# shenzebang/PDE-inverse-problem

Hardware: AMD Instinct MI355X
Metric: particle-steps/sec + achieved HBM GB/s; recovered-drift L2 error (higher is better)
Workload: dtype f32; 1 GPU; C2 kinetic OU d=4: EM simulate (traj+tau+last, fused moments) + KFP residual value_and_grad; dim=4, n_steps=100, particles_per_gpu=2097152, particles_total=2097152, parallelism=dp1

## Files before the change

include/pdeinv.h:

```cpp
#ifndef PDEINV_H
#define PDEINV_H

#include <stddef.h>
#include <stdint.h>

#ifdef __cplusplus
extern "C" {
#endif

#define PDEINV_ABI_VERSION 10
#define PDEINV_MAX_DIM 16
#define PDEINV_MAX_PARAMS 256

typedef enum {
  PDEINV_OK = 0,
  PDEINV_ERR_INVALID = -1,
  PDEINV_ERR_UNSUPPORTED = -2,
  PDEINV_ERR_HIP = -3
} pdeinv_status;

typedef enum {
  PDEINV_POT_QUADRATIC = 0,
  PDEINV_POT_GMM = 1,
  PDEINV_POT_MEANFIELD_QUADRATIC = 2,
  PDEINV_POT_NONE = 3
} pdeinv_potential_kind;

typedef struct {
  int32_t kind;
  int32_t n_centers;
  float sigma;
  int32_t has_center;
  const float* params;
} pdeinv_potential;

typedef struct {
  int64_t n_particles;
  int64_t particle_offset;
  int32_t dim;
  int32_t n_steps;
  float dt;
  float gamma;
  float noise_scale;
  int32_t random_shift;
  uint64_t seed;
  uint32_t counter_offset;
  int64_t ld_z0;
  pdeinv_potential potential;
  const float* d_noise;
  const float* d_shift_u;
  const float* d_meanfield;
} pdeinv_sde_desc;

int pdeinv_moment_len(int m);
size_t pdeinv_sde_workspace_bytes(const pdeinv_sde_desc* desc);
int pdeinv_sde_simulate(const pdeinv_sde_desc* desc, const float* d_z0, float* d_traj,
                        float* d_tau, float* d_last, void* d_workspace, double* d_moments,
                        void* stream);

size_t pdeinv_mf_workspace_bytes(const pdeinv_sde_desc* desc);
int pdeinv_mf_step(const pdeinv_sde_desc* desc, int32_t s, const float* d_z, float* d_z_out,
                   float* d_tau_row, const float* d_tau0, const double* d_xbar_sum,
                   void* d_workspace, double* d_xsum, void* stream);
int64_t pdeinv_mf_sums_len(const pdeinv_sde_desc* desc);
size_t pdeinv_mf_sums_workspace_bytes(const pdeinv_sde_desc* desc);
int pdeinv_mf_sums(const pdeinv_sde_desc* desc, const float* d_z0, void* d_workspace, double* d_sums,
                   void* stream);
int pdeinv_mf_mean_path(const pdeinv_sde_desc* desc, const double* d_sums, float* d_xbar, double* d_xsum,
                        void* stream);
size_t pdeinv_sde_simulate_mf_next_workspace_bytes(const pdeinv_sde_desc* desc);
int pdeinv_sde_simulate_mf_next(const pdeinv_sde_desc* desc, const float* d_z0, float* d_traj, float* d_tau,
                                float* d_last, const pdeinv_sde_desc* next, const float* d_z0_next,
                                void* d_workspace, double* d_sums_next, void* stream);
size_t pdeinv_sde_simulate_mf_kmv_workspace_bytes(const pdeinv_sde_desc* desc, int32_t with_next);
int pdeinv_sde_simulate_mf_kmv(const pdeinv_sde_desc* desc, const float* d_z0, float* d_traj, float* d_tau,
                               float* d_last, float gamma, const float* d_coef, double* d_mom, double* d_wstats,
                               const pdeinv_sde_desc* next, const float* d_z0_next, double* d_sums_next,
                               void* d_workspace, void* stream);
int pdeinv_sde_tau0(const pdeinv_sde_desc* desc, float* d_tau0, void* stream);

size_t pdeinv_moments_workspace_bytes(int64_t n_rows, int32_t m);
int pdeinv_moments(const float* d_z, int64_t n_rows, int32_t m, int64_t ld, void* d_workspace,
                   double* d_out, void* stream);

enum {
  PDEINV_KFP_LOSS = 0,
  PDEINV_KFP_LOSS_GT = 1,
  PDEINV_KFP_GRAD_NORM = 2,
  PDEINV_KFP_NABLA = 3,
  PDEINV_KFP_HESSIAN = 4,
  PDEINV_KFP_FRICTION = 5,
  PDEINV_KFP_NABLA_TRUE = 6,
  PDEINV_KFP_INITIAL = 7,
  PDEINV_KFP_TERMINAL = 8,
  PDEINV_KFP_NOUT = 9
};

typedef struct {
  int32_t dim;
  float gamma;
  float total_time;
  const float* tilde_F;
} pdeinv_kfp_quad_desc;

int pdeinv_residual_kfp_quadratic(const pdeinv_kfp_quad_desc* desc, const double* d_moments,
                                  const float* d_theta, float* d_out, float* d_grad,
                                  void* stream);

enum {
  PDEINV_GMM_ACC_LOSS = 0,
  PDEINV_GMM_ACC_LOSS_GT = 1,
  PDEINV_GMM_ACC_NABLA = 2,
  PDEINV_GMM_ACC_HESSIAN = 3,
  PDEINV_GMM_ACC_FRICTION = 4,
  PDEINV_GMM_ACC_NABLA_TRUE = 5,
  PDEINV_GMM_ACC_INITIAL = 6,
  PDEINV_GMM_ACC_TERMINAL = 7,
  PDEINV_GMM_NACC = 8
};

typedef struct {
  int32_t dim;
  int32_t n_centers;
  float sigma;
  int32_t n_centers_true;
  float sigma_true;
  const float* mus_true;
  float gamma;
  float c_nabla, c_hess, c_fric, c_true, c_init, c_term;
} pdeinv_kfp_gmm_desc;

size_t pdeinv_residual_kfp_gmm_workspace_bytes(const pdeinv_kfp_gmm_desc* desc, int64_t n_init,
                                               int64_t n_term, int64_t n_0T);
int pdeinv_residual_kfp_gmm(const pdeinv_kfp_gmm_desc* desc, const float* d_init,
                            int64_t n_init, int64_t ld_init, const float* d_term,
                            int64_t n_term, int64_t ld_term, const float* d_0T, int64_t n_0T,
                            int64_t ld_0T, const float* d_mus, void* d_workspace,
                            double* d_acc, void* stream);

size_t pdeinv_sde_simulate_kfp_gmm_workspace_bytes(const pdeinv_sde_desc* desc, const pdeinv_kfp_gmm_desc* res);
int pdeinv_sde_simulate_kfp_gmm(const pdeinv_sde_desc* desc, const pdeinv_kfp_gmm_desc* res, const float* d_mus,
// ... 175 lines not shown
```

pde-inverse-problem_amd/csrc/sde.hip:

```cpp
#include <math.h>
#include <stddef.h>
#include <stdlib.h>

#include <type_traits>

#include "sde_common.h"

namespace pdeinv {


template <int D>
__device__ __forceinline__ void grad_quadratic(const SdeArgs& a, const float* q, float* g) {
  if constexpr (D * D + D > 32) {
    kfloat* P = kernarg_params();
#pragma unroll
    for (int r = 0; r < D; ++r) {
      float acc = -P[D * D + r];
#pragma unroll
      for (int c = 0; c < D; ++c) acc = fmaf(P[r * D + c], q[c], acc);
      g[r] = acc;
    }
  } else {
#pragma unroll
    for (int r = 0; r < D; ++r) {
      float acc = -a.params[D * D + r];
#pragma unroll
      for (int c = 0; c < D; ++c) acc = fmaf(a.params[r * D + c], q[c], acc);
      g[r] = acc;
    }
  }
}

template <int D, int KM>
struct GmmCentres {
  GmmPairs<D, KM> g;
  __device__ __forceinline__ void load(const SdeArgs& a) {
#pragma unroll
    for (int p = 0; p < KM / 2; ++p) {
#pragma unroll
      for (int i = 0; i < D; ++i) {
        g.mu[p][i] = f32x2{2 * p < a.K ? a.params[2 * p * D + i] : 0.f, 2 * p + 1 < a.K ? a.params[(2 * p + 1) * D + i] : 0.f};
        asm volatile("" : "+v"(g.mu[p][i]));
      }
      g.c[p] = f32x2{2 * p < a.K ? a.params[kMaxGmmK * D + 2 * p] : -INFINITY,
                     2 * p + 1 < a.K ? a.params[kMaxGmmK * D + 2 * p + 1] : -INFINITY};
      asm volatile("" : "+v"(g.c[p]));
    }
  }
};




template <int D>
__device__ __forceinline__ void store_rows_staged(float* wave_dst, const float* z, float* slot,
                                                  int lane, int n_valid) {
  constexpr int M = 2 * D;
  static_assert(M % 4 == 0, "staged stores need 2d % 4 == 0");
#pragma unroll
  for (int k = 0; k < M; k += 4)
    *reinterpret_cast<f32x4*>(slot + lane * M + k) = f32x4{z[k], z[k + 1], z[k + 2], z[k + 3]};
  __builtin_amdgcn_wave_barrier();
  f32x4 v[M / 4];
#pragma unroll
  for (int k = 0; k < M / 4; ++k) v[k] = *reinterpret_cast<const f32x4*>(slot + 4 * (k * 64 + lane));
  if (n_valid == kWave) {
#pragma unroll
    for (int k = 0; k < M / 4; ++k)
      __builtin_nontemporal_store(v[k], reinterpret_cast<f32x4*>(wave_dst + 4 * (k * 64 + lane)));
  } else {
#pragma unroll
    for (int k = 0; k < M / 4; ++k) {
      const int c = k * 64 + lane;
      if (4 * c < n_valid * M) __builtin_nontemporal_store(v[k], reinterpret_cast<f32x4*>(wave_dst + 4 * c));
    }
  }
  __builtin_amdgcn_wave_barrier();
}

template <int D>
__device__ __forceinline__ void load_rows_staged(const float* wave_src, float* z, float* slot, int lane,
                                                 int n_valid) {
  constexpr int M = 2 * D;
  static_assert(M % 4 == 0, "staged loads need 2d % 4 == 0");
#pragma unroll
  for (int k = 0; k < M / 4; ++k) {
// ... 187 lines not shown
  const float sh_dt = sqrtf(a.dt) * a.ns;
  for (int s = 1; s < a.n_steps; ++s) {
    update(a.dt, sh_dt, (uint32_t)s);
    if (tr) put(tr + (int64_t)s * tr_stride);
    if (active && ta) __builtin_nontemporal_store(tau_value(tau0, s, a.dt), ta + (int64_t)s * a.N);
    if constexpr (MOM) acc.add(z);
  }

  update(h_last, sqrtf(h_last) * a.ns, (uint32_t)a.n_steps);
  if (active && last) store_row<D, kStoreNT>(last + i * M, z);
  if constexpr (NXT) {
    float* red = stage;
    const int wv = threadIdx.x >> 6;
    constexpr int NE = (128 * D + kBlock - 1) / kBlock;
    float v[NE];
#pragma unroll
    for (int t = 0; t < NE; ++t) v[t] = 0.f;
#pragma unroll
    for (int pass = 0; pass < 2; ++pass) {
      const int j0 = 2 * pass, nj = pass ? 1 : 2;
      __syncthreads();
#pragma unroll
      for (int jj = 0; jj < 2; ++jj)
        if (jj < nj) {
#pragma unroll
          for (int k = 0; k < D; ++k) red[((wv * kWave + lane) * 2 + jj) * D + k] = nacc[j0 + jj][k];
        }
      __syncthreads();
#pragma unroll
      for (int t = 0; t < NE; ++t) {
        const int e = threadIdx.x + t * kBlock;
        if (e < nx.np1 * D) {
          const int sp = e / D, k = e - sp * D;
          const int l0 = (64 * sp) / nx.np1, l1 = (64 * sp + 63) / nx.np1;
          for (int w2 = 0; w2 < kWavesPerBlock; ++w2)
            for (int l = l0; l <= l1; ++l) {
              const int jj = sp - ((l * nx.np1) >> 6) - j0;
              if (jj >= 0 && jj < nj) v[t] += red[((w2 * kWave + l) * 2 + jj) * D + k];
            }
        }
      }
    }
#pragma unroll
    for (int t = 0; t < NE; ++t) {
      const int e = threadIdx.x + t * kBlock;
      if (e < nx.np1 * D) nx.partials[(int64_t)e * nb + bid] = v[t];
    }
  }
  if constexpr (RES) {
    res_add(z, z, 2);
    constexpr int NR = PDEINV_GMM_NACC + KR * D;
    float flat[NR];
#pragma unroll
    for (int c = 0; c < PDEINV_GMM_NACC; ++c) flat[c] = racc[c];
    gmm_adjoint_flat<D, KR>(radj, lmod.mu, flat + PDEINV_GMM_NACC);
    __shared__ float rlds[kWavesPerBlock * NR];
    block_reduce_to_slab(flat, PDEINV_GMM_NACC + rf.K * D, rlds, partials, bid, nb);
  }

  if constexpr (MOM) {
    float mv[L];
    acc.finish((float)a.n_steps, w, mv);
    block_reduce_to_slab(mv, L, lds, partials + (int64_t)L * nb, bid, nb);
    MomentAcc<M> term;
    term.zero();
    term.add(z, w);
    block_reduce_to_slab(term.v, L, lds, partials + (int64_t)2 * L * nb, bid, nb);
  }
}

template <typename F>
struct first_param;
template <typename R, typename A0, typename... As>
struct first_param<R (*)(A0, As...)> {
  using type = A0;
};
static_assert(std::is_standard_layout<SdeArgs>::value, "kernarg_params(): SdeArgs must be standard-layout");
static_assert(std::is_same<first_param<decltype(&sde_simulate_kernel<4, PDEINV_POT_QUADRATIC, false, 2>)>::type,
                           SdeArgs>::value &&
                  std::is_same<first_param<decltype(&sde_simulate_kernel<8, PDEINV_POT_MEANFIELD_QUADRATIC, false, 2>)>::type,
                               SdeArgs>::value,
              "kernarg_params() reads SdeArgs::params at its kernarg offset: SdeArgs must stay the first parameter "
              "of sde_simulate_kernel");

template <int D>
__global__ __launch_bounds__(kBlock) void mf_step_kernel(SdeArgs a, int s, float tau0,
                                                         const float* __restrict__ zin,
                                                         float* __restrict__ zout,
                                                         float* __restrict__ tau_row,
                                                         const double* __restrict__ xbar_sum,
                                                         float* __restrict__ partials) {
  constexpr int M = 2 * D;
  constexpr bool kStaged = (M % 4 == 0);
  const int64_t i_raw = (int64_t)blockIdx.x * kBlock + threadIdx.x;
  const bool active = i_raw < a.N;
  const int64_t i = active ? i_raw : a.N - 1;
  const uint64_t gid = (uint64_t)(a.poff + i);
  const int lane = threadIdx.x & (kWave - 1);
  const int64_t wave_row0 = i_raw - lane;
  const int n_valid = (int)((a.N - wave_row0) < kWave ? (a.N - wave_row0) : kWave);
  __shared__ float stage[kStaged ? kBlock * M : 1];
  float* slot = stage + (threadIdx.x - lane) * M;
  float z[M] = {};
  if constexpr (kStaged) {
    if (n_valid > 0) load_rows_staged<D>(zin + wave_row0 * M, z, slot, lane, n_valid);
  } else {
#pragma unroll
    for (int k = 0; k < M; ++k) z[k] = zin[i * M + k];
  }
  const double cnt = xbar_sum[0];
  float y[D];
#pragma unroll
  for (int k = 0; k < D; ++k) y[k] = z[k] - (float)(xbar_sum[1 + k] / cnt);
  float g[D];
#pragma unroll
  for (int r = 0; r < D; ++r) {
    float acc = 0.f;
#pragma unroll
    for (int c = 0; c < D; ++c) acc = fmaf(a.params[r * D + c], y[c], acc);
    g[r] = acc;
  }
  float xi[D];
  if (a.noise) gen_normals<D, true>(a, (uint32_t)gid, (uint32_t)(gid >> 32), (uint32_t)s, i, xi);
  else gen_normals<D, false>(a, (uint32_t)gid, (uint32_t)(gid >> 32), (uint32_t)s, i, xi);
  const float h = (s == 0) ? tau0 : ((s == a.n_steps) ? a.dt - tau0 : a.dt);
  const float sh = sqrtf(h) * a.ns;
  const float gh = a.gamma * h;
#pragma unroll
  for (int k = 0; k < D; ++k) {
    const float p = z[D + k];
    const float pn = fmaf(-gh, p, fmaf(sh, xi[k], fmaf(-h, g[k], p)));
    z[D + k] = pn;
    z[k] = fmaf(h, pn, z[k]);
  }
  if constexpr (kStaged) {
    if (n_valid > 0) store_rows_staged<D>(zout + wave_row0 * M, z, slot, lane, n_valid);
  } else if (active) {
    store_row<D, kStoreNT>(zout + i * M, z);
  }
  if (active && tau_row) tau_row[i] = tau_value(tau0, s, a.dt);
  float v[1 + D];
  v[0] = active ? 1.f : 0.f;
#pragma unroll
  for (int k = 0; k < D; ++k) v[1 + k] = active ? z[k] : 0.f;
  __shared__ float lds[kWavesPerBlock * (1 + D)];
  block_reduce_to_slab(v, 1 + D, lds, partials, blockIdx.x, gridDim.x);
}

__global__ void tau0_kernel(SdeArgs a, float* __restrict__ out) {
  const int64_t i = (int64_t)blockIdx.x * kBlock + threadIdx.x;
  if (i >= a.N) return;
  const uint64_t gid = (uint64_t)(a.poff + i);
  out[i] = a.random_shift ? shift_u(a, (uint32_t)gid, (uint32_t)(gid >> 32), i) * a.dt : 0.f;
}


static int sim_grid(int64_t N) { return grid_for(N); }

}

using namespace pdeinv;

extern "C" int pdeinv_moment_len(int m) { return moment_len(m); }

extern "C" size_t pdeinv_sde_workspace_bytes(const pdeinv_sde_desc* d) {
  if (!d || d->dim < 1 || d->dim > 8 || d->n_particles <= 0) return 0;
  return (size_t)3 * moment_len(2 * d->dim) * sim_grid(d->n_particles) * sizeof(float);
}

template <int D, int POT, bool MOM, int KM = 1>
static void launch_sim(const SdeArgs& a, const float* z0, float* traj, float* tau, float* last,
                       float* ws, hipStream_t st) {
  const dim3 g(sim_grid(a.N)), b(kBlock);
  if (a.noise)
    hipLaunchKernelGGL((sde_simulate_kernel<D, POT, MOM, kStoreStaged, KM, true>), g, b, 0, st, a, z0, traj, tau,
                       last, ws);
  else
    hipLaunchKernelGGL((sde_simulate_kernel<D, POT, MOM, kStoreStaged, KM, false>), g, b, 0, st, a, z0, traj, tau,
                       last, ws);
}

template <int D> constexpr int kResMinWaves = D <= 4 ? 3 : 1;

template <int D, int KM>
static void launch_sim_res(const SdeArgs& a, const GmmResFused& rf, const float* z0, float* traj, float* tau,
                           float* last, float* ws, hipStream_t st) {
  const dim3 g(sim_grid(a.N)), b(kBlock);
  constexpr int W = kResMinWaves<D>;
  if (a.noise)
    hipLaunchKernelGGL((sde_simulate_kernel<D, PDEINV_POT_GMM, false, kStoreStaged, KM, true, W, true>), g, b, 0, st,
                       a, z0, traj, tau, last, ws, rf);
  else
    hipLaunchKernelGGL((sde_simulate_kernel<D, PDEINV_POT_GMM, false, kStoreStaged, KM, false, W, true>), g, b, 0,
                       st, a, z0, traj, tau, last, ws, rf);
}

template <int D, bool MOM>
static void launch_gmm_sim(const SdeArgs& a, const float* z0, float* traj, float* tau, float* last, float* ws,
                           hipStream_t st) {
  if (a.K <= 4) launch_sim<D, PDEINV_POT_GMM, MOM, 4>(a, z0, traj, tau, last, ws, st);
  else if (a.K <= 8) launch_sim<D, PDEINV_POT_GMM, MOM, 8>(a, z0, traj, tau, last, ws, st);
  else launch_sim<D, PDEINV_POT_GMM, MOM, 16>(a, z0, traj, tau, last, ws, st);
}

template <int D>
static int dispatch_sim(const SdeArgs& a, int pot, bool mom, const float* z0, float* traj,
                        float* tau, float* last, float* ws, hipStream_t st) {
  if (pot == PDEINV_POT_MEANFIELD_QUADRATIC) {
    launch_sim<D, PDEINV_POT_MEANFIELD_QUADRATIC, false>(a, z0, traj, tau, last, ws, st);
    return 0;
  }
  if (pot == PDEINV_POT_GMM) {
    if constexpr (D <= 8) {
      if (mom) { launch_gmm_sim<D, true>(a, z0, traj, tau, last, ws, st); return 0; }
    }
    launch_gmm_sim<D, false>(a, z0, traj, tau, last, ws, st);
  } else {
    if constexpr (D <= 8) {
      if (mom) { launch_sim<D, PDEINV_POT_QUADRATIC, true>(a, z0, traj, tau, last, ws, st); return 0; }
    }
    launch_sim<D, PDEINV_POT_QUADRATIC, false>(a, z0, traj, tau, last, ws, st);
  }
  return 0;
}



extern "C" int pdeinv_sde_simulate(const pdeinv_sde_desc* d, const float* z0, float* traj,
                                   float* tau, float* last, void* ws, double* moments,
                                   void* stream) {
  SdeArgs a;
  int rc = build_args(d, a);
  if (rc) return rc;
  const int D = d->dim;
  const bool mom = moments != nullptr;
  if (d->potential.kind == PDEINV_POT_MEANFIELD_QUADRATIC) {
    PDEINV_REQUIRE(d->d_meanfield != nullptr, PDEINV_ERR_INVALID,
                   "sde: McKean–Vlasov needs d_meanfield (pdeinv_mf_mean_path) or pdeinv_mf_step");
    PDEINV_REQUIRE(d->d_shift_u == nullptr, PDEINV_ERR_INVALID,
                   "sde: McKean–Vlasov draws its shared tau0 from the stream (shift_u unsupported)");
    PDEINV_REQUIRE(!mom, PDEINV_ERR_UNSUPPORTED, "sde: fused KFP moments are not defined for McKean–Vlasov");
    a.xbar = d->d_meanfield;
    a.tau0_mf = shared_tau0_host(a, d);
  }
  PDEINV_REQUIRE(!mom || D <= 8, PDEINV_ERR_UNSUPPORTED, "sde: fused moments need dim <= 8");
  hipStream_t st = (hipStream_t)stream;
  const int L = moment_len(2 * D);
  if (a.N == 0) {
    if (mom && hipMemsetAsync(moments, 0, sizeof(double) * 3 * L, st) != hipSuccess)
      return fail(PDEINV_ERR_HIP, "sde: hipMemsetAsync failed");
    return PDEINV_OK;
  }
  PDEINV_REQUIRE(z0 != nullptr, PDEINV_ERR_INVALID, "sde: z0 is null");
  PDEINV_REQUIRE(!mom || ws != nullptr, PDEINV_ERR_INVALID, "sde: moments need a workspace");
  const size_t va = (D % 2 == 0) ? 16 : 8;
  PDEINV_REQUIRE(aligned(traj, va) && aligned(last, va) && aligned(tau, 4), PDEINV_ERR_INVALID,
                 "sde: traj/last must be 16-byte (even dim) or 8-byte (odd dim) aligned");
  float* wsf = (float*)ws;
  switch (D) {
#define CASE(DD) case DD: dispatch_sim<DD>(a, d->potential.kind, mom, z0, traj, tau, last, wsf, st); break;
    CASE(1) CASE(2) CASE(3) CASE(4) CASE(5) CASE(6) CASE(7) CASE(8) CASE(10) CASE(12) CASE(16)
#undef CASE
    default:
      return fail(PDEINV_ERR_UNSUPPORTED, "sde: dim must be one of 1-8, 10, 12, 16");
  }
  rc = check_launch("sde_simulate_kernel");
  if (rc) return rc;
  if (mom) {
    launch_slab_reduce(wsf, sim_grid(a.N), 3 * L, moments, st);
    rc = check_launch("slab_reduce_kernel");
  }
  return rc;
}

static int gmm_res_km(int K) { return K <= 4 ? 4 : (K <= 8 ? 8 : 16); }

extern "C" size_t pdeinv_sde_simulate_kfp_gmm_workspace_bytes(const pdeinv_sde_desc* d, const pdeinv_kfp_gmm_desc* r) {
  if (!d || !r || d->dim < 1 || d->dim > 8 || d->n_particles <= 0 || r->n_centers < 1) return 0;
  return (size_t)(PDEINV_GMM_NACC + r->n_centers * d->dim) * sim_grid(d->n_particles) * sizeof(float);
}

extern "C" int pdeinv_sde_simulate_kfp_gmm(const pdeinv_sde_desc* d, const pdeinv_kfp_gmm_desc* r, const float* mus,
                                           const float* z0, float* traj, float* tau, float* last, void* ws, double* acc,
                                           void* stream) {
  SdeArgs a;
  int rc = build_args(d, a);
  if (rc) return rc;
  PDEINV_REQUIRE(r != nullptr, PDEINV_ERR_INVALID, "sde_kfp_gmm: null residual descriptor");
  const int D = d->dim;
  PDEINV_REQUIRE(d->potential.kind == PDEINV_POT_GMM, PDEINV_ERR_INVALID, "sde_kfp_gmm: the simulated potential must be GMM");
  PDEINV_REQUIRE(r->dim == D, PDEINV_ERR_INVALID, "sde_kfp_gmm: residual dim != simulator dim");
  PDEINV_REQUIRE(D <= 8, PDEINV_ERR_UNSUPPORTED, "sde_kfp_gmm: dim must be <= 8");
  PDEINV_REQUIRE(r->n_centers >= 1 && r->n_centers <= kMaxGmmK && r->n_centers * D <= 64, PDEINV_ERR_UNSUPPORTED,
                 "sde_kfp_gmm: need 1 <= model n_centers <= 16 and n_centers * dim <= 64");
  bool same = r->n_centers_true == d->potential.n_centers && r->sigma_true == d->potential.sigma && r->mus_true;
  for (int k = 0; same && k < r->n_centers_true * D; ++k) same = r->mus_true[k] == d->potential.params[k];
  PDEINV_REQUIRE(same, PDEINV_ERR_INVALID, "sde_kfp_gmm: the residual's true GMM must be the simulated potential");
  PDEINV_REQUIRE(std::isfinite(r->sigma) && r->sigma > 0.f, PDEINV_ERR_INVALID, "sde_kfp_gmm: model sigma must be > 0");
  hipStream_t st = (hipStream_t)stream;
  PDEINV_REQUIRE(acc != nullptr, PDEINV_ERR_INVALID, "sde_kfp_gmm: acc is null");
  if (a.N == 0) {
    if (hipMemsetAsync(acc, 0, sizeof(double) * (PDEINV_GMM_NACC + r->n_centers * D), st) != hipSuccess)
      return fail(PDEINV_ERR_HIP, "sde_kfp_gmm: hipMemsetAsync failed");
    return PDEINV_OK;
  }
  PDEINV_REQUIRE(z0 && mus && ws, PDEINV_ERR_INVALID, "sde_kfp_gmm: null pointer");
  const size_t va = (D % 2 == 0) ? 16 : 8;
  PDEINV_REQUIRE(aligned(traj, va) && aligned(last, va) && aligned(tau, 4), PDEINV_ERR_INVALID,
                 "sde_kfp_gmm: traj/last must be 16-byte (even dim) or 8-byte (odd dim) aligned");
  GmmResFused rf{};
  rf.mus = mus;
  rf.K = r->n_centers;
  rf.s2 = 1.f / (r->sigma * r->sigma);
  rf.l2s = rf.s2 * 1.4426950408889634f;
  rf.c_nabla = r->c_nabla; rf.c_hess = r->c_hess; rf.c_fric = r->c_fric; rf.c_true = r->c_true;
  rf.c_init = r->c_init; rf.c_term = r->c_term;
  rf.inv_ni = 1.f / (float)a.N;
  rf.inv_nt = 1.f / (float)a.N;
  const int km = gmm_res_km(a.K > rf.K ? a.K : rf.K);
  float* wsf = (float*)ws;
  switch (D) {
#define CASE(DD)                                                                          \
  case DD:                                                                                \
    if (km == 4) launch_sim_res<DD, 4>(a, rf, z0, traj, tau, last, wsf, st);              \
    else if (km == 8) launch_sim_res<DD, 8>(a, rf, z0, traj, tau, last, wsf, st);         \
    else launch_sim_res<DD, 16>(a, rf, z0, traj, tau, last, wsf, st);                     \
    break;
    CASE(1) CASE(2) CASE(3) CASE(4) CASE(5) CASE(6) CASE(7) CASE(8)
#undef CASE
    default:
      return fail(PDEINV_ERR_UNSUPPORTED, "sde_kfp_gmm: dim must be in [1, 8]");
  }
  rc = check_launch("sde_simulate_kernel<GMM, fused residual>");
  if (rc) return rc;
  launch_slab_reduce(wsf, sim_grid(a.N), PDEINV_GMM_NACC + r->n_centers * D, acc, st);
  return check_launch("slab_reduce_kernel");
}

extern "C" size_t pdeinv_mf_workspace_bytes(const pdeinv_sde_desc* d) {
  if (!d || d->dim < 1 || d->dim > PDEINV_MAX_DIM || d->n_particles <= 0) return 0;
  return (size_t)(1 + d->dim) * sim_grid(d->n_particles) * sizeof(float);
// ... 287 lines not shown
```

pde-inverse-problem_amd/utils/native.py:

```python
from __future__ import annotations

import ctypes
import math
import os
import subprocess
from typing import Optional

import numpy as np
import torch

_PKG_DIR = os.path.dirname(os.path.dirname(os.path.abspath(__file__)))
CSRC_DIR = os.path.join(_PKG_DIR, "csrc")
LIB_PATH = os.path.join(_PKG_DIR, "_build", "libpdeinv.so")

PDEINV_OK, PDEINV_ERR_INVALID, PDEINV_ERR_UNSUPPORTED, PDEINV_ERR_HIP = 0, -1, -2, -3
POT_QUADRATIC, POT_GMM, POT_MEANFIELD_QUADRATIC, POT_NONE = 0, 1, 2, 3
MAX_DIM, MAX_PARAMS = 16, 256
KFP_NOUT = 9
KFP_SLOTS = ("loss", "loss ground truth", "grad_norm", "loss_nabla", "loss_Hessian",
             "loss_friction", "loss_nabla_true", "loss_initial", "loss_terminal")
GMM_NACC = 8
GMM_ACC_SLOTS = ("loss", "loss_gt", "nabla", "hessian", "friction", "nabla_true", "initial", "terminal")
SQRT2 = math.sqrt(2.0)

ABI_VERSION = 10

EXPORTED_SYMBOLS = (
    "pdeinv_moment_len", "pdeinv_sde_workspace_bytes", "pdeinv_sde_simulate",
    "pdeinv_sde_simulate_mf_kmv_workspace_bytes", "pdeinv_sde_simulate_mf_kmv",
    "pdeinv_mf_workspace_bytes", "pdeinv_mf_step", "pdeinv_sde_tau0",
    "pdeinv_moments_workspace_bytes", "pdeinv_moments", "pdeinv_residual_kfp_quadratic",
    "pdeinv_residual_kfp_gmm_workspace_bytes", "pdeinv_residual_kfp_gmm",
    "pdeinv_residual_kfp_gmm_finalize", "pdeinv_gmm_potential", "pdeinv_gaussian_sample",
    "pdeinv_gaussian_sample_grouped", "pdeinv_fp_rows", "pdeinv_fp_exact_sample",
    "pdeinv_philox_fill", "pdeinv_gather_subsample", "pdeinv_abi_version", "pdeinv_last_error",
    "pdeinv_runtime_version", "pdeinv_moments_batched_workspace_bytes", "pdeinv_moments_batched",
    "pdeinv_kmv_weights_workspace_bytes", "pdeinv_kmv_weights", "pdeinv_residual_kmv",
    "pdeinv_residual_kmv_workspace_bytes",
    "pdeinv_mlp_param_count", "pdeinv_rocblas_calls", "pdeinv_residual_kfp_mlp_workspace_bytes", "pdeinv_residual_kfp_mlp",
    "pdeinv_kfp_terms_finalize", "pdeinv_gather_random_step", "pdeinv_mlp_fused_supported",
    "pdeinv_adam_update", "pdeinv_realnvp_param_count", "pdeinv_realnvp_logdensity",
    "pdeinv_realnvp_grad_workspace", "pdeinv_realnvp_value_and_grad",
    "pdeinv_residual_kmv_mlp_workspace_bytes", "pdeinv_residual_kmv_mlp", "pdeinv_kmv_mlp_path",
    "pdeinv_mf_sums_len", "pdeinv_mf_sums_workspace_bytes", "pdeinv_mf_sums", "pdeinv_mf_mean_path",
    "pdeinv_kmv_moments_weights_workspace_bytes", "pdeinv_kmv_moments_weights",
    "pdeinv_kmv_moments_weights_mf_sums_workspace_bytes", "pdeinv_kmv_moments_weights_mf_sums",
    "pdeinv_sde_simulate_kfp_gmm_workspace_bytes", "pdeinv_sde_simulate_kfp_gmm",
    "pdeinv_sde_simulate_mf_next_workspace_bytes", "pdeinv_sde_simulate_mf_next", "pdeinv_ou_exact_sample",
)


class PotentialDesc(ctypes.Structure):
    _fields_ = [("kind", ctypes.c_int32), ("n_centers", ctypes.c_int32), ("sigma", ctypes.c_float),
                ("has_center", ctypes.c_int32), ("params", ctypes.c_void_p)]


class SdeDesc(ctypes.Structure):
    _fields_ = [("n_particles", ctypes.c_int64), ("particle_offset", ctypes.c_int64),
                ("dim", ctypes.c_int32), ("n_steps", ctypes.c_int32), ("dt", ctypes.c_float),
                ("gamma", ctypes.c_float), ("noise_scale", ctypes.c_float),
                ("random_shift", ctypes.c_int32), ("seed", ctypes.c_uint64),
                ("counter_offset", ctypes.c_uint32), ("ld_z0", ctypes.c_int64),
                ("potential", PotentialDesc), ("d_noise", ctypes.c_void_p),
                ("d_shift_u", ctypes.c_void_p), ("d_meanfield", ctypes.c_void_p)]


class KfpQuadDesc(ctypes.Structure):
    _fields_ = [("dim", ctypes.c_int32), ("gamma", ctypes.c_float), ("total_time", ctypes.c_float),
                ("tilde_F", ctypes.c_void_p)]


class KmvDesc(ctypes.Structure):
    _fields_ = [("dim", ctypes.c_int32), ("n_sets", ctypes.c_int32), ("gamma", ctypes.c_float),
                ("tilde_F", ctypes.c_void_p)]


class KfpMlpDesc(ctypes.Structure):
    _fields_ = [("dim", ctypes.c_int32), ("n_layers", ctypes.c_int32), ("width", ctypes.c_int32),
                ("out_features", ctypes.c_int32), ("true_kind", ctypes.c_int32), ("n_centers_true", ctypes.c_int32),
                ("sigma_true", ctypes.c_float), ("true_params", ctypes.c_void_p), ("gamma", ctypes.c_float),
                ("c_nabla", ctypes.c_float), ("c_hess", ctypes.c_float), ("c_fric", ctypes.c_float),
                ("c_true", ctypes.c_float), ("c_init", ctypes.c_float), ("c_term", ctypes.c_float),
                ("chunk_rows", ctypes.c_int64), ("impl", ctypes.c_int32), ("boundary_value", ctypes.c_int32)]


class OuDesc(ctypes.Structure):
    _fields_ = [("n", ctypes.c_int32), ("taylor_degree", ctypes.c_int32), ("squarings", ctypes.c_int32),
                ("t_min", ctypes.c_double), ("t_max", ctypes.c_double), ("d_powers", ctypes.c_void_p),
                ("d_m0", ctypes.c_void_p), ("d_P0", ctypes.c_void_p)]


class KmvMlpDesc(ctypes.Structure):
    _fields_ = [("dim", ctypes.c_int32), ("n_layers", ctypes.c_int32), ("width", ctypes.c_int32),
                ("out_features", ctypes.c_int32), ("n_sets", ctypes.c_int32), ("n_rows", ctypes.c_int64),
                ("gamma", ctypes.c_float), ("tilde_F", ctypes.c_void_p), ("chunk_rows", ctypes.c_int64),
                ("impl", ctypes.c_int32)]


MLP_IMPL_AUTO, MLP_IMPL_LIBRARY, MLP_IMPL_FUSED, MLP_IMPL_PAIRS_RING = 0, 1, 2, 3

ACTIVATIONS = {"celu": 0, "relu": 1, "tanh": 2, "elu": 3, "silu": 4, "softplus": 5, "gelu": 6}


class RealNvpDesc(ctypes.Structure):
    _fields_ = [("dim", ctypes.c_int32), ("n_layers", ctypes.c_int32), ("embed_time_dim", ctypes.c_int32),
                ("ignore_time", ctypes.c_int32), ("soft_init", ctypes.c_float), ("activation", ctypes.c_int32),
                ("masks", ctypes.c_void_p), ("base_mean", ctypes.c_void_p), ("base_inv_cov", ctypes.c_void_p),
                ("base_log_det", ctypes.c_float)]


class KfpGmmDesc(ctypes.Structure):
    _fields_ = [("dim", ctypes.c_int32), ("n_centers", ctypes.c_int32), ("sigma", ctypes.c_float),
                ("n_centers_true", ctypes.c_int32), ("sigma_true", ctypes.c_float),
                ("mus_true", ctypes.c_void_p), ("gamma", ctypes.c_float),
                ("c_nabla", ctypes.c_float), ("c_hess", ctypes.c_float), ("c_fric", ctypes.c_float),
                ("c_true", ctypes.c_float), ("c_init", ctypes.c_float), ("c_term", ctypes.c_float)]


_lib = None


def build(force: bool = False, jobs: int = 8) -> str:
    args = ["make", "-C", CSRC_DIR, f"-j{jobs}"]
    if force:
        subprocess.check_call(["make", "-C", CSRC_DIR, "clean"])
    subprocess.check_call(args)
    return LIB_PATH


def lib():
    global _lib
    if _lib is not None:
        return _lib
    path = os.environ.get("PDEINV_LIBRARY", LIB_PATH)
    if not os.path.exists(path):
        raise RuntimeError(f"pdeinv native library missing at {path}; run __graft_entry__.build() "
                           "(the hot path has no CPU fallback)")
    L = ctypes.CDLL(path)
    P, i32, i64, u32, u64, f32 = (ctypes.c_void_p, ctypes.c_int32, ctypes.c_int64, ctypes.c_uint32,
                                  ctypes.c_uint64, ctypes.c_float)
    sig = {
        "pdeinv_moment_len": (i32, [i32]),
        "pdeinv_sde_workspace_bytes": (ctypes.c_size_t, [P]),
        "pdeinv_sde_simulate": (i32, [P, P, P, P, P, P, P, P]),
        "pdeinv_mf_workspace_bytes": (ctypes.c_size_t, [P]),
        "pdeinv_mf_step": (i32, [P, i32, P, P, P, P, P, P, P, P]),
        "pdeinv_sde_tau0": (i32, [P, P, P]),
        "pdeinv_sde_simulate_kfp_gmm_workspace_bytes": (ctypes.c_size_t, [P, P]),
        "pdeinv_sde_simulate_kfp_gmm": (i32, [P, P, P, P, P, P, P, P, P, P]),
        "pdeinv_mf_sums_len": (i64, [P]),
        "pdeinv_mf_sums_workspace_bytes": (ctypes.c_size_t, [P]),
        "pdeinv_sde_simulate_mf_next_workspace_bytes": (ctypes.c_size_t, [P]),
        "pdeinv_sde_simulate_mf_next": (i32, [P, P, P, P, P, P, P, P, P, P]),
        "pdeinv_sde_simulate_mf_kmv_workspace_bytes": (ctypes.c_size_t, [P, i32]),
        "pdeinv_sde_simulate_mf_kmv": (i32, [P, P, P, P, P, f32, P, P, P, P, P, P, P, P]),
        "pdeinv_mf_sums": (i32, [P, P, P, P, P]),
        "pdeinv_mf_mean_path": (i32, [P, P, P, P, P]),
        "pdeinv_kmv_moments_weights_workspace_bytes": (ctypes.c_size_t, [i64, i64, i32]),
        "pdeinv_kmv_moments_weights": (i32, [i32, f32, P, P, i64, i64, i64, i64, P, P, P, P]),
        "pdeinv_kmv_moments_weights_mf_sums_workspace_bytes": (ctypes.c_size_t, [i64, i64, i32, P]),
        "pdeinv_kmv_moments_weights_mf_sums": (i32, [i32, f32, P, P, i64, i64, i64, i64, P, P, P, P, P, P, P]),
        "pdeinv_moments_workspace_bytes": (ctypes.c_size_t, [i64, i32]),
        "pdeinv_moments": (i32, [P, i64, i32, i64, P, P, P]),
        "pdeinv_residual_kfp_quadratic": (i32, [P, P, P, P, P, P]),
        "pdeinv_residual_kfp_gmm_workspace_bytes": (ctypes.c_size_t, [P, i64, i64, i64]),
        "pdeinv_residual_kfp_gmm": (i32, [P, P, i64, i64, P, i64, i64, P, i64, i64, P, P, P, P]),
        "pdeinv_residual_kfp_gmm_finalize": (i32, [P, P, P, P, P]),
        "pdeinv_gmm_potential": (i32, [i32, i32, f32, P, P, i64, i64, P, P, P]),
        "pdeinv_gaussian_sample": (i32, [i64, i32, u64, u32, i64, P, P, P, P]),
        "pdeinv_gaussian_sample_grouped": (i32, [i64, i64, i32, u64, u32, i64, P, P, P, P]),
        "pdeinv_ou_exact_sample": (i32, [P, i64, i64, u64, u32, u32, i64, P, P, P, P, P, P]),
        "pdeinv_philox_fill": (i32, [u64, u32, u32, i64, P, P]),
        "pdeinv_gather_subsample": (i32, [P, i64, i32, i32, P, i64, P, i32, P, P]),
        "pdeinv_abi_version": (i32, []),
        "pdeinv_last_error": (ctypes.c_char_p, []),
        "pdeinv_runtime_version": (i32, []),
        "pdeinv_moments_batched_workspace_bytes": (ctypes.c_size_t, [i64, i64, i32]),
        "pdeinv_moments_batched": (i32, [P, i64, i64, i32, i64, i64, P, P, P]),
        "pdeinv_kmv_weights_workspace_bytes": (ctypes.c_size_t, [i64, i64, i32]),
        "pdeinv_kmv_weights": (i32, [i32, f32, P, P, i64, i64, i64, i64, P, P, P, P]),
        "pdeinv_residual_kmv_workspace_bytes": (ctypes.c_size_t, [P]),
        "pdeinv_residual_kmv": (i32, [P, P, P, P, P, P, P, P]),
        "pdeinv_mlp_param_count": (i64, [i32, i32, i32, i32]),
        "pdeinv_rocblas_calls": (i64, []),
        "pdeinv_mlp_fused_supported": (i32, [i32, i32, i32, i32]),
        "pdeinv_adam_update": (i32, [P, P, P, P, i64, f32, f32, f32, f32, f32, i32, P]),
        "pdeinv_realnvp_param_count": (i64, [P]),
        "pdeinv_realnvp_logdensity": (i32, [P, P, P, i64, P, i64, i64, P, P]),
        "pdeinv_realnvp_grad_workspace": (i64, [P, i64]),
        "pdeinv_realnvp_value_and_grad": (i32, [P, P, P, i64, P, i64, i64, P, P, P, i64, P]),
        "pdeinv_residual_kfp_mlp_workspace_bytes": (ctypes.c_size_t, [P]),
        "pdeinv_residual_kfp_mlp": (i32, [P, P, i64, i64, P, i64, i64, P, i64, i64, P, P, P, P, P]),
        "pdeinv_kfp_terms_finalize": (i32, [P, P, i64, f32, P, P]),
        "pdeinv_residual_kmv_mlp_workspace_bytes": (ctypes.c_size_t, [P]),
        "pdeinv_kmv_mlp_path": (ctypes.c_int, [P]),
        "pdeinv_residual_kmv_mlp": (i32, [P, P, i64, i64, P, P, P, P, P, P]),
        "pdeinv_gather_random_step": (i32, [P, i64, i32, i32, u64, u32, P, P, P]),
        "pdeinv_fp_rows": (i32, [P, i64, i64, i32, i32, P, P]),
        "pdeinv_fp_exact_sample": (i32, [i64, i32, u64, u32, i64, f32, f32, P, P, P, P, P, P, P, P]),
    }
    for name, (res, args) in sig.items():
        fn = getattr(L, name)
        fn.restype = res
        fn.argtypes = args
    if L.pdeinv_abi_version() != ABI_VERSION:
        raise RuntimeError("libpdeinv ABI version mismatch")
    _lib = L
    return _lib


def _check(rc: int, what: str) -> None:
    if rc == PDEINV_OK:
        return
    msg = f"{what}: {lib().pdeinv_last_error().decode(errors='replace')}"
    if rc == PDEINV_ERR_INVALID:
        raise ValueError(msg)
    if rc == PDEINV_ERR_UNSUPPORTED:
        raise NotImplementedError(msg)
    raise RuntimeError(msg)


def _require_gpu():
    if not torch.cuda.is_available():
        raise RuntimeError("pdeinv hot path needs a ROCm GPU (no CPU fallback)")


def _dev(t: Optional[torch.Tensor], name: str, dtype=torch.float32) -> Optional[ctypes.c_void_p]:
# ... 26 lines not shown
    return np.ascontiguousarray(np.asarray(a, dtype=np.float32).ravel())


def make_potential(kind: int, params=None, n_centers: int = 0, sigma: float = 1.0,
                   has_center: bool = False):
    host = _host_f32(np.zeros(1) if params is None else params)
    desc = PotentialDesc(kind, int(n_centers), float(sigma), int(has_center),
                         host.ctypes.data_as(ctypes.c_void_p))
    return desc, host


def _sim_desc(z0: torch.Tensor, n_steps: int, dt: float, gamma: float, potential: dict, seed: int,
              counter_offset: int, particle_offset: int, noise_scale: float, random_shift: bool,
              noise: Optional[torch.Tensor], shift_u: Optional[torch.Tensor]):
    if z0.dim() != 2 or z0.shape[1] % 2:
        raise ValueError("q0_p0 must be [N, 2d]")
    N, m = z0.shape
    d = m // 2
    p_desc, p_host = make_potential(**potential)
    desc = SdeDesc()
    desc.n_particles = N
    desc.particle_offset = int(particle_offset)
    desc.dim = d
    desc.n_steps = int(n_steps)
    desc.dt = float(dt)
    desc.gamma = float(gamma)
    desc.noise_scale = float(noise_scale)
    desc.random_shift = int(bool(random_shift))
    desc.seed = int(seed) & 0xFFFFFFFFFFFFFFFF
    desc.counter_offset = int(counter_offset) & 0xFFFFFFFF
    z0p, _, ld = _rows(z0, "q0_p0", m) if N > 0 else (None, 0, m)
    desc.ld_z0 = ld
    desc.potential = p_desc
    if noise is not None:
        if tuple(noise.shape) != (n_steps + 1, N, d) or not noise.is_contiguous():
            raise ValueError(f"noise must be contiguous [{n_steps + 1}, {N}, {d}]")
        desc.d_noise = _dev(noise, "noise")
    if shift_u is not None:
        if tuple(shift_u.shape) != (N,) or not shift_u.is_contiguous():
            raise ValueError(f"shift_u must be contiguous [{N}]")
        desc.d_shift_u = _dev(shift_u, "shift_u")
    return desc, p_host, z0p


def _sim_outputs(res: dict, z0: torch.Tensor, n_steps: int, traj: bool, tau: bool, last: bool) -> dict:
    N, m = z0.shape
    dev = z0.device
    if traj and "traj" not in res:
        res["traj"] = torch.empty((n_steps, N, m), device=dev, dtype=torch.float32)
    if tau and "tau" not in res:
        res["tau"] = torch.empty((n_steps, N), device=dev, dtype=torch.float32)
    if last and "last" not in res:
        res["last"] = torch.empty((N, m), device=dev, dtype=torch.float32)
    return res


def sde_simulate(z0: torch.Tensor, n_steps: int, dt: float, gamma: float, potential: dict, *,
                 seed: int, counter_offset: int = 0, particle_offset: int = 0,
                 noise_scale: float = SQRT2, random_shift: bool = True,
                 noise: Optional[torch.Tensor] = None, shift_u: Optional[torch.Tensor] = None,
                 traj: bool = True, tau: bool = True, last: bool = True,
                 moments: bool = False, out: Optional[dict] = None) -> dict:
    _require_gpu()
    desc, p_host, z0p = _sim_desc(z0, n_steps, dt, gamma, potential, seed, counter_offset, particle_offset,
                                  noise_scale, random_shift, noise, shift_u)
    m = z0.shape[1]
    res = _sim_outputs({} if out is None else out, z0, n_steps, traj, tau, last)
    ws = None
    if moments:
        if "moments" not in res:
            res["moments"] = torch.empty((3, moment_len(m)), device=z0.device, dtype=torch.float64)
        nbytes = lib().pdeinv_sde_workspace_bytes(ctypes.byref(desc))
        ws = torch.empty(max(nbytes // 4, 1), device=z0.device, dtype=torch.float32)
    rc = lib().pdeinv_sde_simulate(
        ctypes.byref(desc), z0p, _dev(res.get("traj") if traj else None, "traj"),
        _dev(res.get("tau") if tau else None, "tau"), _dev(res.get("last") if last else None, "last"),
        _dev(ws, "workspace"), _dev(res.get("moments") if moments else None, "moments", torch.float64),
        stream_handle())
    del p_host
    _check(rc, "pdeinv_sde_simulate")
    return res


def sde_simulate_kfp_gmm(z0: torch.Tensor, n_steps: int, dt: float, gamma: float, potential: dict, res_desc,
                         mus: torch.Tensor, *, seed: int, counter_offset: int = 0, particle_offset: int = 0,
                         noise_scale: float = SQRT2, random_shift: bool = True, noise: Optional[torch.Tensor] = None,
                         shift_u: Optional[torch.Tensor] = None, traj: bool = True, tau: bool = True,
                         last: bool = True, out: Optional[dict] = None) -> dict:
    _require_gpu()
    desc, p_host, z0p = _sim_desc(z0, n_steps, dt, gamma, potential, seed, counter_offset, particle_offset,
                                  noise_scale, random_shift, noise, shift_u)
    rdesc, _keep = res_desc
    K, d = rdesc.n_centers, rdesc.dim
    if tuple(mus.shape) != (K, d):
        raise ValueError(f"mus must be [{K}, {d}]")
    mus_c = mus.contiguous()
    res = _sim_outputs({} if out is None else out, z0, n_steps, traj, tau, last)
    nbytes = lib().pdeinv_sde_simulate_kfp_gmm_workspace_bytes(ctypes.byref(desc), ctypes.byref(rdesc))
    ws = torch.empty(max(nbytes // 4, 1), device=z0.device, dtype=torch.float32)
    res["acc"] = torch.empty(GMM_NACC + K * d, device=z0.device, dtype=torch.float64)
    rc = lib().pdeinv_sde_simulate_kfp_gmm(
        ctypes.byref(desc), ctypes.byref(rdesc), _dev(mus_c, "mus"), z0p,
        _dev(res.get("traj") if traj else None, "traj"), _dev(res.get("tau") if tau else None, "tau"),
        _dev(res.get("last") if last else None, "last"), _dev(ws, "workspace"), _dev(res["acc"], "acc", torch.float64),
        stream_handle())
    del p_host
    _check(rc, "pdeinv_sde_simulate_kfp_gmm")
    return res


def sde_tau0(N: int, dt: float, *, seed: int, counter_offset: int = 0, particle_offset: int = 0,
             random_shift: bool = True, device="cuda") -> torch.Tensor:
    _require_gpu()
    desc = SdeDesc()
    desc.n_particles = N
    desc.particle_offset = particle_offset
    desc.dim = 1
    desc.n_steps = 1
    desc.dt = dt
    desc.noise_scale = SQRT2
    desc.random_shift = int(random_shift)
    desc.seed = seed
    desc.counter_offset = counter_offset
    desc.potential = PotentialDesc(POT_NONE, 0, 1.0, 0, None)
    out = torch.empty(N, device=device, dtype=torch.float32)
    _check(lib().pdeinv_sde_tau0(ctypes.byref(desc), _dev(out, "tau0"), stream_handle()), "pdeinv_sde_tau0")
    return out


def mf_sums(desc: SdeDesc, z0: torch.Tensor) -> torch.Tensor:
    _require_gpu()
    L = int(lib().pdeinv_mf_sums_len(ctypes.byref(desc)))
    if L <= 0:
        raise ValueError("mf_sums: bad descriptor")
    if z0.dim() != 2 or z0.shape[0] != desc.n_particles or z0.shape[1] != 2 * desc.dim:
        raise ValueError(f"mf_sums: z0 must be [{desc.n_particles}, {2 * desc.dim}]")
    if z0.shape[0] and z0.stride(1) != 1:
        raise ValueError("mf_sums: z0 must have unit inner stride")
    desc.ld_z0 = z0.stride(0) if z0.shape[0] > 1 else 2 * desc.dim
    ws = torch.empty(max(int(lib().pdeinv_mf_sums_workspace_bytes(ctypes.byref(desc))) // 4, 1), device=z0.device,
                     dtype=torch.float32)
    out = torch.empty(L, device=z0.device, dtype=torch.float64)
    _check(lib().pdeinv_mf_sums(ctypes.byref(desc), _dev(z0, "z0") if z0.shape[0] else None, _dev(ws, "ws"),
                                _dev(out, "sums", torch.float64), stream_handle()), "pdeinv_mf_sums")
    return out


def mf_mean_path(desc: SdeDesc, sums: torch.Tensor, xsum: bool = True):
    _require_gpu()
    n, d = desc.n_steps, desc.dim
    xbar = torch.empty((n + 1, d), device=sums.device, dtype=torch.float32)
    xs = torch.empty((n + 2, 1 + d), device=sums.device, dtype=torch.float64) if xsum else None
    _check(lib().pdeinv_mf_mean_path(ctypes.byref(desc), _dev(sums, "sums", torch.float64), _dev(xbar, "xbar"),
                                     _dev(xs, "xsum", torch.float64), stream_handle()), "pdeinv_mf_mean_path")
    return xbar, xs


def sde_simulate_desc(desc: SdeDesc, z0: torch.Tensor, traj: Optional[torch.Tensor], tau: Optional[torch.Tensor],
                      last: Optional[torch.Tensor]) -> None:
    _require_gpu()
    N, m, n = desc.n_particles, 2 * desc.dim, desc.n_steps
    for t, shape, name in ((traj, (n, N, m), "traj"), (tau, (n, N), "tau"), (last, (N, m), "last")):
        if t is not None and (tuple(t.shape) != shape or not t.is_contiguous()):
            raise ValueError(f"{name} must be contiguous {shape}")
    if N and (z0.dim() != 2 or tuple(z0.shape) != (N, m) or z0.stride(1) != 1):
        raise ValueError(f"z0 must be [{N}, {m}] with unit inner stride")
# ... 608 lines not shown
```

Before: 145.0 billion particle-steps/s.

## Add resident multi-group SDE kernel keeping G particle groups per wave in registers

Adds a dim-4 quadratic-potential kernel where each wave owns G groups of 64 particles. It keeps their state in registers across all time steps, caches tau0 in LDS, and does one moment reduction per block instead of per wave. An auto schedule selects it when there are enough waves per CU, and a new API lets callers force either path. The aim is to amortize per-wave setup, RNG and reduction overhead and to raise memory-level parallelism. The cost is higher register pressure (launch bounds with 2 min blocks at G=16) and fewer blocks in the grid.

New measurement: 142.5 billion particle-steps/s. -1.7%, worse.

```diff
diff --git a/include/pdeinv.h b/include/pdeinv.h
--- a/include/pdeinv.h
+++ b/include/pdeinv.h
@@ -57,6 +57,10 @@
 int pdeinv_sde_simulate(const pdeinv_sde_desc* desc, const float* d_z0, float* d_traj,
                         float* d_tau, float* d_last, void* d_workspace, double* d_moments,
                         void* stream);
+#define PDEINV_SCHEDULE_AUTO 0
+#define PDEINV_SCHEDULE_PER_WAVE 1
+#define PDEINV_SCHEDULE_RESIDENT 2
+int pdeinv_sde_set_schedule(int32_t mode);
 
 size_t pdeinv_mf_workspace_bytes(const pdeinv_sde_desc* desc);
 int pdeinv_mf_step(const pdeinv_sde_desc* desc, int32_t s, const float* d_z, float* d_z_out,
diff --git a/pde-inverse-problem_amd/csrc/sde.hip b/pde-inverse-problem_amd/csrc/sde.hip
--- a/pde-inverse-problem_amd/csrc/sde.hip
+++ b/pde-inverse-problem_amd/csrc/sde.hip
@@ -2,6 +2,7 @@
 #include <stddef.h>
 #include <stdlib.h>
 
+#include <atomic>
 #include <type_traits>
 
 #include "sde_common.h"
@@ -355,6 +356,157 @@
                                SdeArgs>::value,
               "kernarg_params() reads SdeArgs::params at its kernarg offset: SdeArgs must stay the first parameter "
               "of sde_simulate_kernel");
+
+#ifndef PDEINV_RESIDENT_G
+#define PDEINV_RESIDENT_G 16
+#endif
+constexpr int kResidentG = PDEINV_RESIDENT_G;
+#ifndef PDEINV_RESIDENT_ILP
+#define PDEINV_RESIDENT_ILP 1
+#endif
+constexpr int kResidentIlp = PDEINV_RESIDENT_ILP;
+#ifndef PDEINV_RESIDENT_TAU16
+#define PDEINV_RESIDENT_TAU16 0
+#endif
+constexpr bool kResidentTau16 = PDEINV_RESIDENT_TAU16 != 0;
+template <int G> constexpr int kResidentMinBlocks = G >= 16 ? 2 : (G >= 8 ? 3 : 4);
+
+template <int D, int G, bool MOM>
+__global__ __launch_bounds__(kBlock, kResidentMinBlocks<G>) void sde_resident_kernel(SdeArgs a, const float* __restrict__ z0,
+                                                                               float* __restrict__ traj,
+                                                                               float* __restrict__ tau,
+                                                                               float* __restrict__ last,
+                                                                               float* __restrict__ partials) {
+  constexpr int M = 2 * D;
+  constexpr int L = moment_len(M);
+  static_assert(M % 4 == 0 && D * D + D <= 32, "resident schedule: staged stores, A and b in SGPRs");
+  const int bid = a.remap ? xcd_block(blockIdx.x, gridDim.x) : (int)blockIdx.x;
+  const int nb = gridDim.x;
+  const int lane = threadIdx.x & (kWave - 1);
+  const int wv = __builtin_amdgcn_readfirstlane((int)(threadIdx.x >> 6));
+  const int64_t wave_row0 = ((int64_t)bid * kWavesPerBlock + wv) * (G * kWave);
+
+  __shared__ __attribute__((aligned(16))) float stage[kBlock * M];
+  __shared__ __attribute__((aligned(16))) float tau0_s[kBlock * G];
+  __shared__ float lds[kWavesPerBlock * L];
+  float* slot = stage + wv * (kWave * M);
+  float* t0 = tau0_s + wv * (G * kWave) + lane;
+
+  auto rows_valid = [&](int64_t row0) {
+    const int64_t r = a.N - row0;
+    return (int)(r < kWave ? (r > 0 ? r : 0) : kWave);
+  };
+
+  float z[G][M];
+  [[maybe_unused]] MomentAcc<M> init;
+  if constexpr (MOM) init.zero();
+  int n_act = 0;
+#pragma unroll
+  for (int g = 0; g < G; ++g) {
+    int64_t row0 = wave_row0 + g * kWave;
+    asm volatile("" : "+s"(row0));
+    const bool act = lane < rows_valid(row0);
+    float tau0 = 0.f;
+#pragma unroll
+    for (int k = 0; k < M; ++k) z[g][k] = 0.f;
+    if (act) {
+      const int64_t i = row0 + lane;
+#pragma unroll
+      for (int k = 0; k < M; ++k) z[g][k] = z0[i * a.ld_z0 + k];
+      const uint64_t gid = (uint64_t)(a.poff + i);
+      if (a.random_shift) tau0 = shift_u(a, (uint32_t)gid, (uint32_t)(gid >> 32), i) * a.dt;
+    }
+    t0[g * kWave] = tau0;
+    n_act += act ? 1 : 0;
+    if constexpr (MOM) init.add(z[g], act ? 1.f : 0.f);
+  }
+  if constexpr (MOM) block_reduce_to_slab(init.v, L, lds, partials, bid, nb);
+
+  PairGram<(MOM ? M : 2)> acc;
+  acc.zero();
+  const float sh_dt = sqrtf(a.dt) * a.ns;
+  static_assert(!kResidentTau16 || G % 4 == 0, "tau16 stores take 4 groups per instruction");
+  const bool tau16 = kResidentTau16 && tau != nullptr && wave_row0 + G * kWave <= a.N && (a.N & 3) == 0 &&
+                     ((uintptr_t)tau & 15) == 0;
+  if constexpr (kResidentTau16) __builtin_amdgcn_wave_barrier();
+
+  auto update = [&](float (&zg)[M], int64_t row0, bool act, float h, float sh, int s) {
+    h = act ? h : 0.f;
+    sh = act ? sh : 0.f;
+    const uint64_t gid = (uint64_t)(a.poff + row0) + (uint32_t)lane;
+    float gr[D], xi[D];
+    grad_quadratic<D>(a, zg, gr);
+    gen_normals<D, false>(a, (uint32_t)gid, (uint32_t)(gid >> 32), (uint32_t)s, 0, xi);
+    const float gh = a.gamma * h;
+#pragma unroll
+    for (int k = 0; k < D; ++k) {
+      const float p = zg[D + k];
+      const float pn = fmaf(-gh, p, fmaf(sh, xi[k], fmaf(-h, gr[k], p)));
+      zg[D + k] = pn;
+      zg[k] = fmaf(h, pn, zg[k]);
+    }
+  };
+
+  for (int s = 0; s < a.n_steps; ++s) {
+#pragma unroll
+    for (int g = 0; g < G; ++g) {
+      int64_t row0 = wave_row0 + g * kWave;
+      asm volatile("" : "+s"(row0));
+      const int n_valid = rows_valid(row0);
+      const bool act = lane < n_valid;
+      const float tau0 = t0[g * kWave];
+      float h = a.dt, sh = sh_dt;
+      if (s == 0) {
+        asm volatile("");
+        h = tau0;
+        sh = sqrtf(tau0) * a.ns;
+      }
+      update(z[g], row0, act, h, sh, s);
+      if (traj) store_rows_staged<D>(traj + ((int64_t)s * a.N + row0) * M, z[g], slot, lane, n_valid);
+      if (tau && act && !tau16)
+        __builtin_nontemporal_store(tau_value(tau0, s, a.dt), tau + ((int64_t)s * a.N + row0) + lane);
+      if constexpr (MOM) acc.add(z[g]);
+      if ((g + 1) % kResidentIlp == 0) __builtin_amdgcn_sched_barrier(0);
+    }
+    if constexpr (kResidentTau16) {
+      if (tau16) {
+        const float* tw = tau0_s + wv * (G * kWave);
+        float* dst = tau + ((int64_t)s * a.N + wave_row0);
+#pragma unroll
+        for (int j = 0; j < G / 4; ++j) {
+          const f32x4 t = *reinterpret_cast<const f32x4*>(tw + 4 * (j * kWave + lane));
+          const f32x4 v = {tau_value(t[0], s, a.dt), tau_value(t[1], s, a.dt), tau_value(t[2], s, a.dt),
+                           tau_value(t[3], s, a.dt)};
+          __builtin_nontemporal_store(v, reinterpret_cast<f32x4*>(dst + 4 * (j * kWave + lane)));
+        }
+      }
+    }
+  }
+#pragma unroll
+  for (int g = 0; g < G; ++g) {
+    int64_t row0 = wave_row0 + g * kWave;
+    asm volatile("" : "+s"(row0));
+    const int n_valid = rows_valid(row0);
+    const float h_last = a.dt - t0[g * kWave];
+    update(z[g], row0, lane < n_valid, h_last, sqrtf(h_last) * a.ns, a.n_steps);
+    if (last) store_rows_staged<D>(last + row0 * M, z[g], slot, lane, n_valid);
+    __builtin_amdgcn_sched_barrier(0);
+  }
+
+  if constexpr (MOM) {
+    float mv[L];
+    acc.finish((float)(a.n_steps * n_act), 1.f, mv);
+    block_reduce_to_slab(mv, L, lds, partials + (int64_t)L * nb, bid, nb);
+    MomentAcc<M> term;
+    term.zero();
+#pragma unroll
+    for (int g = 0; g < G; ++g) {
+      const bool act = lane < rows_valid(wave_row0 + g * kWave);
+      term.add(z[g], act ? 1.f : 0.f);
+    }
+    block_reduce_to_slab(term.v, L, lds, partials + (int64_t)2 * L * nb, bid, nb);
+  }
+}
 
 template <int D>
 __global__ __launch_bounds__(kBlock) void mf_step_kernel(SdeArgs a, int s, float tau0,
@@ -430,11 +582,49 @@
 
 static int sim_grid(int64_t N) { return grid_for(N); }
 
+static std::atomic<int32_t> g_schedule{PDEINV_SCHEDULE_AUTO};
+
+static int resident_grid(int64_t N) { return grid_for(N, (int64_t)kBlock * kResidentG); }
+
+static bool resident_applies(const pdeinv_sde_desc* d) {
+  return d->dim == 4 && d->d_noise == nullptr &&
+         (d->potential.kind == PDEINV_POT_QUADRATIC || d->potential.kind == PDEINV_POT_NONE);
+}
+
+static int device_cu_count() {
+  static std::atomic<int> cached[64];
+  int dev = 0;
+  if (hipGetDevice(&dev) != hipSuccess || dev < 0 || dev >= 64) return 0;
+  int n = cached[dev].load(std::memory_order_relaxed);
+  if (n == 0) {
+    if (hipDeviceGetAttribute(&n, hipDeviceAttributeMultiprocessorCount, dev) != hipSuccess) n = 0;
+    cached[dev].store(n, std::memory_order_relaxed);
+  }
+  return n;
+}
+
+constexpr int kResidentAutoWavesPerCu = 4;
+static bool use_resident(const pdeinv_sde_desc* d) {
+  if (!resident_applies(d)) return false;
+  const int32_t mode = g_schedule.load(std::memory_order_relaxed);
+  if (mode == PDEINV_SCHEDULE_PER_WAVE) return false;
+  if (mode == PDEINV_SCHEDULE_RESIDENT) return true;
+  const int cus = device_cu_count();
+  const int64_t waves = (d->n_particles + (int64_t)kWave * kResidentG - 1) / ((int64_t)kWave * kResidentG);
+  return cus > 0 && waves >= (int64_t)kResidentAutoWavesPerCu * cus;
+}
+
 }
 
 using namespace pdeinv;
 
 extern "C" int pdeinv_moment_len(int m) { return moment_len(m); }
+
+extern "C" int pdeinv_sde_set_schedule(int32_t mode) {
+  PDEINV_REQUIRE(mode >= PDEINV_SCHEDULE_AUTO && mode <= PDEINV_SCHEDULE_RESIDENT, PDEINV_ERR_INVALID,
+                 "sde_set_schedule: mode must be 0 (auto), 1 (per-wave) or 2 (resident)");
+  return g_schedule.exchange(mode);
+}
 
 extern "C" size_t pdeinv_sde_workspace_bytes(const pdeinv_sde_desc* d) {
   if (!d || d->dim < 1 || d->dim > 8 || d->n_particles <= 0) return 0;
@@ -530,6 +720,22 @@
   PDEINV_REQUIRE(aligned(traj, va) && aligned(last, va) && aligned(tau, 4), PDEINV_ERR_INVALID,
                  "sde: traj/last must be 16-byte (even dim) or 8-byte (odd dim) aligned");
   float* wsf = (float*)ws;
+  if (use_resident(d)) {
+    const int nb = resident_grid(a.N);
+    if (mom)
+      hipLaunchKernelGGL((sde_resident_kernel<4, kResidentG, true>), dim3(nb), dim3(kBlock), 0, st, a, z0, traj, tau,
+                         last, wsf);
+    else
+      hipLaunchKernelGGL((sde_resident_kernel<4, kResidentG, false>), dim3(nb), dim3(kBlock), 0, st, a, z0, traj, tau,
+                         last, wsf);
+    rc = check_launch("sde_resident_kernel");
+    if (rc) return rc;
+    if (mom) {
+      launch_slab_reduce(wsf, nb, 3 * L, moments, st);
+      rc = check_launch("slab_reduce_kernel");
+    }
+    return rc;
+  }
   switch (D) {
 #define CASE(DD) case DD: dispatch_sim<DD>(a, d->potential.kind, mom, z0, traj, tau, last, wsf, st); break;
     CASE(1) CASE(2) CASE(3) CASE(4) CASE(5) CASE(6) CASE(7) CASE(8) CASE(10) CASE(12) CASE(16)
diff --git a/pde-inverse-problem_amd/utils/native.py b/pde-inverse-problem_amd/utils/native.py
--- a/pde-inverse-problem_amd/utils/native.py
+++ b/pde-inverse-problem_amd/utils/native.py
@@ -1,5 +1,6 @@
 from __future__ import annotations
 
+import contextlib
 import ctypes
 import math
 import os
@@ -26,7 +27,7 @@
 ABI_VERSION = 10
 
 EXPORTED_SYMBOLS = (
-    "pdeinv_moment_len", "pdeinv_sde_workspace_bytes", "pdeinv_sde_simulate",
+    "pdeinv_moment_len", "pdeinv_sde_workspace_bytes", "pdeinv_sde_simulate", "pdeinv_sde_set_schedule",
     "pdeinv_sde_simulate_mf_kmv_workspace_bytes", "pdeinv_sde_simulate_mf_kmv",
     "pdeinv_mf_workspace_bytes", "pdeinv_mf_step", "pdeinv_sde_tau0",
     "pdeinv_moments_workspace_bytes", "pdeinv_moments", "pdeinv_residual_kfp_quadratic",
@@ -143,6 +144,7 @@
         "pdeinv_moment_len": (i32, [i32]),
         "pdeinv_sde_workspace_bytes": (ctypes.c_size_t, [P]),
         "pdeinv_sde_simulate": (i32, [P, P, P, P, P, P, P, P]),
+        "pdeinv_sde_set_schedule": (i32, [i32]),
         "pdeinv_mf_workspace_bytes": (ctypes.c_size_t, [P]),
         "pdeinv_mf_step": (i32, [P, i32, P, P, P, P, P, P, P, P]),
         "pdeinv_sde_tau0": (i32, [P, P, P]),
@@ -335,6 +337,25 @@
     return res
 
 
+SCHEDULE_AUTO, SCHEDULE_PER_WAVE, SCHEDULE_RESIDENT = 0, 1, 2
+
+
+def sde_set_schedule(mode: int) -> int:
+    prev = lib().pdeinv_sde_set_schedule(int(mode))
+    if prev < 0:
+        _check(prev, "pdeinv_sde_set_schedule")
+    return prev
+
+
+@contextlib.contextmanager
+def sde_schedule(mode: int):
+    prev = sde_set_schedule(mode)
+    try:
+        yield
+    finally:
+        sde_set_schedule(prev)
+
+
 def sde_simulate_kfp_gmm(z0: torch.Tensor, n_steps: int, dt: float, gamma: float, potential: dict, res_desc,
                          mus: torch.Tensor, *, seed: int, counter_offset: int = 0, particle_offset: int = 0,
                          noise_scale: float = SQRT2, random_shift: bool = True, noise: Optional[torch.Tensor] = None,
```
